# ubc-vision/StableKeypoints

Hardware: AMD Instinct MI355X
Metric: images/sec for token-optimization step (SD1.5, 512^2, K=10 kpts) (higher is better)
Workload: dtype f32 (fp32 MFMA / VALU throughout; flash attention of the >= 1024-key self-attention layers: 3xbf16 operand split, fp32 accumulate, error <= the fp32 kernel's)

## Files before the change

### include/skp.h

```cpp
#ifndef SKP_H
#define SKP_H

#include <stdint.h>

#ifdef __cplusplus
extern "C" {
#endif

#define SKP_MAX_LAYERS 8
#define SKP_MAX_SUBJECTS 4

#define SKP_E_BADARG (-1)
#define SKP_E_RANGE  (-2)
#define SKP_E_LDS    (-3)

int skp_abi_version(void);

int skp_tune_set(const char* key, int value);
int skp_tune_get(const char* key);

int skp_gemm_nt_f32(const float* A, const float* B, float* C, int M, int N, int K, int Z0, int Z1,
                    int64_t sa0, int64_t sa1, int64_t sam, int64_t sak,
                    int64_t sb0, int64_t sb1, int64_t sbn, int64_t sbk,
                    int64_t sc0, int64_t sc1, int64_t scm, float alpha, void* stream);
// ... 32 lines not shown
int skp_unwarp_accumulate_f32(const float* M, const float* theta_inv, int n, int K, int R, int S, float* tot, float* num,
                              int finish, void* stream);

int skp_group_norm_coef_f32(const float* x, const float* off, const float* gamma, const float* beta, float* mean, float* rstd,
                            float* coef, const float* bs, int nblk, int pix, float* workspace, int N, int C, int G, int HW,
                            float eps, void* stream);
int skp_conv3x3_f4_gn_ok(int B, int Cin, int Cout, int H, int W);
int skp_conv3x3_f4_gn_f32(const void* x, const void* U, const void* bias, const void* residual, void* y, float* stats,
                          const float* coef, int B, int Cin, int Cout, int H, int W, void* stream);

int skp_conv3x3_f4r_ok(int B, int Cin, int Cout, int H, int W);
int skp_conv3x3_f4r_filter_f32(const void* w, void* R, int Cout, int Cin, int flip_transpose, void* stream);
int64_t skp_conv3x3_f4r_workspace(int B, int Cin, int Cout, int H, int W);
int skp_conv3x3_f4r_f32(const void* x, const void* R, const void* bias, const void* residual, void* y, void* workspace,
                        int B, int Cin, int Cout, int H, int W, void* stream);

int skp_cross_attn_fwd_f32(const float* q, const float* k, const float* v, float* out, float* lse,
                           int B, int Bk, int H, int N, int T, int d, float scale, void* stream);
int64_t skp_cross_attn_bwd_workspace(int B, int H, int N, int T, int d);
int skp_cross_attn_bwd_f32(const float* q, const float* k, const float* v, const float* out,
                           const float* dout, const float* lse, float* dq, float* dk, float* dv,
                           float* workspace, int B, int Bk, int H, int N, int T, int d, float scale,
                           void* stream);

int skp_text_attn_fwd_ok(int B, int H, int N, int d, int ld);
int skp_text_attn_fwd_f32(const float* q, const float* k, const float* v, float* out,
                          int B, int H, int N, int d, int ld, float scale, void* stream);

int skp_attn_map_bwd_ex_f32(const float* const* S , float* const* dS , const int* s ,
                            int L, int B, int H, int T, int R, const float* dM, const float* lse,
                            float* workspace, float* dot_io, int ldt, int64_t m_bstride, int mode, void* stream);

int64_t skp_flash_attn_bwd_workspace(int B, int Bk, int H, int N, int Nk, int d);
int skp_flash_attn_fwd_f32(const float* q, const float* k, const float* v, float* out, float* lse,
                           int B, int Bk, int H, int N, int Nk, int d, float scale, void* stream);
int skp_flash_attn_bwd_f32(const float* q, const float* k, const float* v, const float* out, const float* dout,
                           const float* lse, float* dq, float* dk, float* dv, float* workspace,
                           int B, int Bk, int H, int N, int Nk, int d, float scale, void* stream);
int skp_flash_attn_bwd_ld_f32(const float* q, const float* k, const float* v, const float* out, const float* dout,
                              const float* lse, float* dq, float* dk, float* dv, float* workspace,
                              int B, int Bk, int H, int N, int Nk, int d, float scale, int ldg, void* stream);

int skp_flash_attn_fwd_split_ok(int B, int Bk, int H, int N, int Nk, int d);
int64_t skp_flash_attn_fwd_split_workspace(int B, int Bk, int H, int N, int Nk, int d);
int skp_flash_attn_fwd_split_f32(const float* q, const float* k, const float* v, float* out, float* lse, void* workspace,
                                 int B, int Bk, int H, int N, int Nk, int d, float scale, void* stream);
// ... 128 lines not shown
```

### stablekeypoints_amd/_native.py

```python
from __future__ import annotations

import ctypes as C
import os

import torch

_HERE = os.path.dirname(os.path.abspath(__file__))
LIB_PATH = os.environ.get("SKP_LIB_PATH") or os.path.join(_HERE, "csrc", "libskp_hip.so")
ABI_VERSION = 44

_vp, _i, _f, _i64 = C.c_void_p, C.c_int, C.c_float, C.c_int64

SIGNATURES = {
    "skp_abi_version": [],
    "skp_tune_set": [C.c_char_p, _i],
    "skp_tune_get": [C.c_char_p],
    "skp_group_norm_onepass_ok": [_i, _i, _i, _i],
    "skp_gemm_nt_f32": [_vp, _vp, _vp, _i, _i, _i, _i, _i,
                        _i64, _i64, _i64, _i64, _i64, _i64, _i64, _i64, _i64, _i64, _i64, _f, _vp],
    "skp_qk_logits_f32": [_vp, _vp, _vp, _i, _i, _i, _i, _i, _i, _f, _vp],
    "skp_attn_map_fwd_f32": [C.POINTER(_vp), C.POINTER(_i), _i, _i, _i, _i, _i, _vp, _vp, _vp],
    "skp_attn_map_fwd_ex_f32": [C.POINTER(_vp), C.POINTER(_i), _i, _i, _i, _i, _i, _vp, _vp, _vp, _i, _i64, _i, _vp],
    "skp_attn_map_bwd_ex_f32": [C.POINTER(_vp), C.POINTER(_vp), C.POINTER(_i), _i, _i, _i, _i, _i, _vp, _vp, _vp, _vp,
                                _i, _i64, _i, _vp],
    "skp_attn_map_bwd_workspace": [C.POINTER(_i), _i, _i, _i, _i, _i],
    "skp_attn_map_bwd_f32": [C.POINTER(_vp), C.POINTER(_vp), C.POINTER(_i), _i, _i, _i, _i, _i, _vp, _vp, _vp, _vp],
    "skp_group_norm_coef_f32": [_vp, _vp, _vp, _vp, _vp, _vp, _vp, _vp, _i, _i, _vp, _i, _i, _i, _i, _f, _vp],
    "skp_conv3x3_f4_gn_ok": [_i, _i, _i, _i, _i],
    "skp_conv3x3_f4_gn_f32": [_vp, _vp, _vp, _vp, _vp, _vp, _vp, _i, _i, _i, _i, _i, _vp],
    "skp_unwarp_accumulate_f32": [_vp, _vp, _i, _i, _i, _i, _vp, _vp, _i, _vp],
    "skp_attn_map_fwd_wide_f32": [C.POINTER(_vp), C.POINTER(_i), _i, _i, _i, _i, _i, _vp, _vp, _vp, _i, _i, _vp],
    "skp_attn_map_fwd_wide_ok": [C.POINTER(_i), _i, _i, _i],
    "skp_attn_map_bwd_col_ok": [C.POINTER(_i), _i, _i, _i, _i, _i],
    "skp_attn_map_bwd_col_workspace": [C.POINTER(_i), _i, _i, _i, _i, _i, _i],
    "skp_attn_map_bwd_col_f32": [C.POINTER(_vp), C.POINTER(_vp), C.POINTER(_i), _i, _i, _i, _i, _i, _vp, _vp, _i, _vp, _vp,
                                 _i, _vp],
    "skp_attn_map_bwd_sparse_workspace": [C.POINTER(_i), _i, _i, _i, _i, _i, _i],
    "skp_attn_map_bwd_sparse_f32": [C.POINTER(_vp), C.POINTER(_vp), C.POINTER(_i), _i, _i, _i, _i, _i, _vp, _vp, _i, _vp, _vp,
                                    _i, _vp],
    "skp_token_stats_f32": [_vp, _i, _i, _i, _f, _f, _vp, _vp, _vp, _vp],
    "skp_select_tokens": [_vp, _vp, _i, _i, _i, _i, _vp, _vp, _vp],
    "skp_select_tokens_batched": [_vp, _vp, _i, _i, _i, _i, _i, _vp, _vp, _vp],
    "skp_losses_fwd_f32": [_vp, _vp, _vp, _i, _i, _i, _vp, _i, _f, C.POINTER(_f), _vp, _vp, _vp, _vp, _vp],
    "skp_losses_fwd_dev_f32": [_vp, _vp, _vp, _i, _i, _i, _vp, _i, _f, _vp, _vp, _vp, _vp, _vp, _vp],
    "skp_rows_axpy_f32": [_vp, _vp, _i, _i64, _vp, _vp, _vp, _vp, _vp],
    "skp_cross_attn_fwd_f32": [_vp, _vp, _vp, _vp, _vp, _i, _i, _i, _i, _i, _i, _f, _vp],
    "skp_cross_attn_bwd_workspace": [_i, _i, _i, _i, _i],
    "skp_cross_attn_bwd_f32": [_vp, _vp, _vp, _vp, _vp, _vp, _vp, _vp, _vp, _vp, _i, _i, _i, _i, _i, _i, _f, _vp],
    "skp_text_attn_fwd_ok": [_i, _i, _i, _i, _i],
    "skp_text_attn_fwd_f32": [_vp, _vp, _vp, _vp, _i, _i, _i, _i, _i, _f, _vp],
    "skp_group_norm_fwd_f32": [_vp, _vp, _vp, _vp, _vp, _vp, _vp, _vp, _i, _i, _i, _i, _f, _i, _vp],
    "skp_group_norm_bwd_f32": [_vp, _vp, _vp, _vp, _vp, _vp, _vp, _vp, _vp, _i, _i, _i, _i, _f, _i, _vp],
    "skp_group_norm_bwd_add_f32": [_vp, _vp, _vp, _vp, _vp, _vp, _vp, _vp, _vp, _vp, _i, _i, _i, _i, _f, _i, _vp],
    "skp_add_bias_residual_f32": [_vp, _vp, _vp, _vp, _i, _i, _i, _vp],
    "skp_add_layer_norm_ok": [_i],
    "skp_add_layer_norm_fwd_f32": [_vp, _vp, _vp, _vp, _vp, _vp, _vp, _i64, _i, _f, _vp],
    "skp_add_layer_norm_bwd_f32": [_vp, _vp, _vp, _vp, _vp, _vp, _i64, _i, _vp],
    "skp_conv3x3_filter_f32": [_vp, _vp, _i, _i, _i, _vp],
    "skp_conv3x3_workspace": [_i, _i, _i, _i, _i, _i],
    "skp_conv3x3_f32": [_vp, _vp, _vp, _vp, _vp, _vp, _i, _i, _i, _i, _i, _i, _vp],
    "skp_conv3x3_f4_filter_f32": [_vp, _vp, _i, _i, _i, _vp],
    "skp_conv3x3_f4_workspace": [_i, _i, _i, _i, _i],
    "skp_conv3x3_f4_f32": [_vp, _vp, _vp, _vp, _vp, _vp, _i, _i, _i, _i, _i, _vp],
    "skp_flash_attn_fwd_split_ok": [_i, _i, _i, _i, _i, _i],
    "skp_flash_attn_fwd_split_workspace": [_i, _i, _i, _i, _i, _i],
    "skp_flash_attn_fwd_split_f32": [_vp, _vp, _vp, _vp, _vp, _vp, _i, _i, _i, _i, _i, _i, C.c_float, _vp],
    "skp_flash_attn_fwd_wide_ok": [_i, _i, _i, _i, _i, _i],
    "skp_flash_attn_fwd_wide_workspace": [_i, _i, _i, _i, _i, _i],
    "skp_flash_attn_fwd_wide_f32": [_vp, _vp, _vp, _vp, _vp, _i, _i, _i, _i, _i, _i, _f, _vp],
    "skp_flash_attn_bwd_split_ok": [_i, _i, _i, _i, _i, _i],
    "skp_flash_attn_bwd_split_workspace": [_i, _i, _i, _i, _i, _i],
# ... 120 lines not shown
```

### stablekeypoints_amd/csrc/skp_common.h

```cpp
#pragma once
#include <hip/hip_runtime.h>
#include <stdint.h>
#include "../../include/skp.h"

#define SKP_WAVE 64
#define SKP_LOG2E 1.4426950408889634f

typedef float f32x16 __attribute__((ext_vector_type(16)));
typedef float f32x4 __attribute__((ext_vector_type(4)));
typedef float f32x2 __attribute__((ext_vector_type(2)));

enum { SKP_TUNE_WINO_SPLIT = 0, SKP_TUNE_WINO_RAW_MAX_TILES, SKP_TUNE_MAP_BANDS, SKP_TUNE_FA2_TWO_KERNEL_BWD, SKP_TUNE_GN_FOLD_MAX_COUT, SKP_TUNE_CROSS_ATTN_TS,
       SKP_TUNE_CONV_S2W, SKP_TUNE_CONV_UP2, SKP_TUNE_COUNT };
int skp_tune(int key);

static inline int skp_launch_status() {
    hipError_t e = hipGetLastError();
    return e == hipSuccess ? 0 : (int)e;
}

__device__ __forceinline__ void skp_cubic_taps(int dst, float ratio, int n, int idx[4], float w[4]) {
    const float A = -0.75f;
    const float src = ratio * ((float)dst + 0.5f) - 0.5f;
    const float fl = floorf(src);
    const float t = src - fl;
    const int i0 = (int)fl;
    float x = t + 1.0f;
    w[0] = ((A * x - 5.0f * A) * x + 8.0f * A) * x - 4.0f * A;
    x = t;
    w[1] = ((A + 2.0f) * x - (A + 3.0f)) * x * x + 1.0f;
    x = 1.0f - t;
    w[2] = ((A + 2.0f) * x - (A + 3.0f)) * x * x + 1.0f;
    x = 2.0f - t;
    w[3] = ((A * x - 5.0f * A) * x + 8.0f * A) * x - 4.0f * A;
#pragma unroll
    for (int i = 0; i < 4; ++i) {
// ... 44 lines not shown
```

### stablekeypoints_amd/csrc/skp_cross_attn.hip

```cpp
#include "skp_attn_tiles.h"

#define SKP_CA_KSPLIT_MAX 16

int skp_gemm_nt_splitk(const float* A, const float* B, float* C, float* partial, int64_t c_elems, int ksplit,
                       int M, int N, int K, int Z0, int Z1,
                       int64_t sa0, int64_t sa1, int64_t sam, int64_t sak,
                       int64_t sb0, int64_t sb1, int64_t sbn, int64_t sbk,
                       int64_t sc0, int64_t sc1, int64_t scm, float alpha, void* stream);

static int ca_ksplit(int N) { int k = N / 256; return k < 1 ? 1 : (k > SKP_CA_KSPLIT_MAX ? SKP_CA_KSPLIT_MAX : k); }

template <int D8, int TT>
__global__ __launch_bounds__(256) void skp_cross_attn_fwd_kernel(const float* __restrict__ q, const float* __restrict__ k,
                                                                 const float* __restrict__ v, float* __restrict__ out,
                                                                 float* __restrict__ lse, int Bk, int H, int N, int T,
                                                                 float scale) {
    using S = CAShape<D8, TT>;
    extern __shared__ __attribute__((aligned(16))) float smem[];
    const int tid = threadIdx.x, wave = tid >> 6, lane = tid & 63, i = lane & 31, hi = lane >> 5;
    const int b = blockIdx.z, h = blockIdx.y, C = H * S::D;
    const int n0 = blockIdx.x * 128 + wave * 32, n = n0 + i;
    const bool nv = n < N;
    const float* qrow = q + ((size_t)b * N + (nv ? n : N - 1)) * C + h * S::D;
    const float sl2 = scale * SKP_LOG2E;
    f32x4 qv[D8];
#pragma unroll
    for (int j = 0; j < D8; ++j) qv[j] = *(const f32x4*)(qrow + 8 * j + 4 * hi) * sl2;
    const size_t kvoff = (Bk == 1 ? 0 : (size_t)b * T * C) + (size_t)h * S::D;
    ca_stage<D8, TT>(smem, k + kvoff, T, C, tid);
    __syncthreads();
    f32x16 acc[TT];
// ... 37 lines not shown
                const int nn = n0 + (r & 3) + 8 * (r >> 2) + 4 * hi;
                if (nn < N) out[((size_t)b * N + nn) * C + h * S::D + c] = o[ct][r];
            }
        }
    }
}

template <int D8, int TT>
__global__ __launch_bounds__(256) void skp_cross_attn_bwd_kernel(const float* __restrict__ q, const float* __restrict__ k,
                                                                 const float* __restrict__ v, const float* __restrict__ out,
                                                                 const float* __restrict__ dout, const float* __restrict__ lse,
                                                                 float* __restrict__ dq, float* __restrict__ Pst,
                                                                 float* __restrict__ dSst, int Bk, int H, int N, int T,
                                                                 float scale) {
    using S = CAShape<D8, TT>;
    extern __shared__ __attribute__((aligned(16))) float smem[];
    const int tid = threadIdx.x, wave = tid >> 6, lane = tid & 63, i = lane & 31, hi = lane >> 5;
    const int b = blockIdx.z, h = blockIdx.y, C = H * S::D;
    const int n0 = blockIdx.x * 128 + wave * 32, n = n0 + i;
    const bool nv = n < N;
    const size_t rowoff = ((size_t)b * N + (nv ? n : N - 1)) * C + h * S::D;
    const float sl2 = scale * SKP_LOG2E;
    const size_t kvoff = (Bk == 1 ? 0 : (size_t)b * T * C) + (size_t)h * S::D;
    ca_stage<D8, TT>(smem, k + kvoff, T, C, tid);
    f32x16 p[TT], dp[TT];
    float dsum = 0.f;
    {
        f32x4 qv[D8];
#pragma unroll
        for (int j = 0; j < D8; ++j) qv[j] = *(const f32x4*)(q + rowoff + 8 * j + 4 * hi) * sl2;
        __syncthreads();
#pragma unroll
        for (int tt = 0; tt < TT; ++tt)
#pragma unroll
            for (int r = 0; r < 16; ++r) p[tt][r] = 0.f;
        ca_swapped_product<D8, TT>(smem, qv, p, i, hi);
    }
    const float lse2 = lse[((size_t)b * H + h) * N + (nv ? n : N - 1)] * SKP_LOG2E;
#pragma unroll
    for (int tt = 0; tt < TT; ++tt)
#pragma unroll
        for (int r = 0; r < 16; ++r)
            p[tt][r] = (ca_tok(tt, r, hi) < T) ? __builtin_amdgcn_exp2f(p[tt][r] - lse2) : 0.f;
    __syncthreads();
    ca_stage<D8, TT>(smem, v + kvoff, T, C, tid);
    {
        f32x4 dov[D8];
#pragma unroll
        for (int j = 0; j < D8; ++j) {
            dov[j] = *(const f32x4*)(dout + rowoff + 8 * j + 4 * hi);
            const f32x4 ov = *(const f32x4*)(out + rowoff + 8 * j + 4 * hi);
            dsum += dov[j][0] * ov[0] + dov[j][1] * ov[1] + dov[j][2] * ov[2] + dov[j][3] * ov[3];
        }
        dsum += __shfl_xor(dsum, 32, 64);
        __syncthreads();
#pragma unroll
        for (int tt = 0; tt < TT; ++tt)
#pragma unroll
            for (int r = 0; r < 16; ++r) dp[tt][r] = 0.f;
        ca_swapped_product<D8, TT>(smem, dov, dp, i, hi);
    }
    const size_t stb = ((size_t)b * H + h) * S::TP * N;
#pragma unroll
    for (int tt = 0; tt < TT; ++tt)
#pragma unroll
        for (int r = 0; r < 16; ++r) {
            dp[tt][r] = p[tt][r] * (dp[tt][r] - dsum);
            if (nv) {
                const size_t o = stb + (size_t)ca_tok(tt, r, hi) * N + n;
                Pst[o] = p[tt][r];
                dSst[o] = dp[tt][r];
            }
        }
    __syncthreads();
    ca_stage<D8, TT>(smem, k + kvoff, T, C, tid);
    __syncthreads();
    f32x16 o[S::CT];
    ca_reg_product<D8, TT>(smem, dp, o, i, hi);
#pragma unroll
    for (int ct = 0; ct < S::CT; ++ct) {
        const int c = ct * 32 + i;
        if (c < S::D) {
#pragma unroll
            for (int r = 0; r < 16; ++r) {
                const int nn = n0 + (r & 3) + 8 * (r >> 2) + 4 * hi;
                if (nn < N) dq[((size_t)b * N + nn) * C + h * S::D + c] = scale * o[ct][r];
            }
        }
    }
}

template <int D8>
struct CATS {
    using S = CAShape<D8, 1>;
    static constexpr int OUT = S::CT * 1024;
    static constexpr int REG = (32 * S::LDK > OUT ? 32 * S::LDK : OUT);
};

template <int D8>
// ... 126 lines not shown
        ca_swapped_product<D8, 1>(reg, qv, p, i, hi);
    }
    const float lse2 = lse[((size_t)b * H + h) * N + (nv ? n : N - 1)] * SKP_LOG2E;
#pragma unroll
    for (int r = 0; r < 16; ++r) p[0][r] = (t0 + ca_tok(0, r, hi) < T) ? __builtin_amdgcn_exp2f(p[0][r] - lse2) : 0.f;
    ca_stage_wave<D8>(reg, v + kvoff, t0, T, C, lane);
    {
        f32x4 dov[D8];
#pragma unroll
        for (int j = 0; j < D8; ++j) {
            dov[j] = *(const f32x4*)(dout + rowoff + 8 * j + 4 * hi);
            const f32x4 ov = *(const f32x4*)(out + rowoff + 8 * j + 4 * hi);
            dsum += dov[j][0] * ov[0] + dov[j][1] * ov[1] + dov[j][2] * ov[2] + dov[j][3] * ov[3];
        }
        dsum += __shfl_xor(dsum, 32, 64);
#pragma unroll
        for (int r = 0; r < 16; ++r) dp[0][r] = 0.f;
        ca_swapped_product<D8, 1>(reg, dov, dp, i, hi);
    }
    const size_t stb = ((size_t)b * H + h) * TP * N;
#pragma unroll
    for (int r = 0; r < 16; ++r) {
        dp[0][r] = p[0][r] * (dp[0][r] - dsum);
        if (nv) {
            const size_t o = stb + (size_t)(t0 + ca_tok(0, r, hi)) * N + n;
            Pst[o] = p[0][r];
            dSst[o] = dp[0][r];
        }
    }
    ca_stage_wave<D8>(reg, k + kvoff, t0, T, C, lane);
    f32x16 o[S::CT];
    ca_reg_product<D8, 1>(reg, dp, o, i, hi);
    ca_merge_store<D8, NW>(smem, reg, o, dq, scale, b, h, H, N, n0, wave, lane);
}

static bool ca_use_ts(int B, int H, int N, int T, int d) {
    if (skp_tune(SKP_TUNE_CROSS_ATTN_TS) == 1) return false;
    const int tt = (T + 31) / 32;
    if (tt < 2 || !(d == 80 || d == 160)) return false;
    return (long)((N + 127) / 128) * H * B * 4 < 1024;
}

static int ca_check(int B, int Bk, int H, int N, int T, int d) {
    if (B <= 0 || H <= 0 || N <= 0 || T <= 0 || d <= 0 || (Bk != 1 && Bk != B)) return SKP_E_BADARG;
    if (T > 128 || B > 65535 || H > 65535) return SKP_E_RANGE;
    if (d != 8 && d != 16 && d != 32 && d != 40 && d != 64 && d != 80 && d != 160) return SKP_E_RANGE;
    return 0;
}

#define SKP_CA_DISPATCH(KERNEL, ...)                                                                     \
    {                                                                                                    \
        const int tt = (T + 31) / 32;                                                                    \
        const int tsel = tt <= 1 ? 1 : (tt <= 3 ? 3 : 4);                                                \
        dim3 grid((N + 127) / 128, H, B), block(256);                                                    \
        hipStream_t st = (hipStream_t)stream;                                                            \
        int launched = 0;                                                                                \
        SKP_CA_CASE(KERNEL, 1, 1, __VA_ARGS__) SKP_CA_CASE(KERNEL, 1, 3, __VA_ARGS__) SKP_CA_CASE(KERNEL, 1, 4, __VA_ARGS__)     \
        SKP_CA_CASE(KERNEL, 2, 1, __VA_ARGS__) SKP_CA_CASE(KERNEL, 2, 3, __VA_ARGS__) SKP_CA_CASE(KERNEL, 2, 4, __VA_ARGS__)     \
        SKP_CA_CASE(KERNEL, 4, 1, __VA_ARGS__) SKP_CA_CASE(KERNEL, 4, 3, __VA_ARGS__) SKP_CA_CASE(KERNEL, 4, 4, __VA_ARGS__)     \
        SKP_CA_CASE(KERNEL, 5, 1, __VA_ARGS__) SKP_CA_CASE(KERNEL, 5, 3, __VA_ARGS__) SKP_CA_CASE(KERNEL, 5, 4, __VA_ARGS__)     \
        SKP_CA_CASE(KERNEL, 8, 1, __VA_ARGS__) SKP_CA_CASE(KERNEL, 8, 3, __VA_ARGS__) SKP_CA_CASE(KERNEL, 8, 4, __VA_ARGS__)     \
        SKP_CA_CASE(KERNEL, 10, 1, __VA_ARGS__) SKP_CA_CASE(KERNEL, 10, 3, __VA_ARGS__) SKP_CA_CASE(KERNEL, 10, 4, __VA_ARGS__)  \
        SKP_CA_CASE(KERNEL, 20, 1, __VA_ARGS__) SKP_CA_CASE(KERNEL, 20, 3, __VA_ARGS__) SKP_CA_CASE(KERNEL, 20, 4, __VA_ARGS__)  \
        if (!launched) return SKP_E_RANGE;                                                               \
    }

#define SKP_CA_CASE(KERNEL, D8V, TTV, ...)                                                               \
    if (!launched && d == D8V * 8 && tsel == TTV) {                                                      \
        const size_t lds = CAShape<D8V, TTV>::LDS_FLOATS * sizeof(float);                                \
        if (lds > 64 * 1024) {                                                                           \
            hipError_t e = hipFuncSetAttribute((const void*)KERNEL<D8V, TTV>,                            \
                                               hipFuncAttributeMaxDynamicSharedMemorySize, (int)lds);    \
            if (e != hipSuccess) return (int)e;                                                          \
        }                                                                                                \
        hipLaunchKernelGGL((KERNEL<D8V, TTV>), grid, block, lds, st, __VA_ARGS__);                       \
        launched = 1;                                                                                    \
    }

#define SKP_CA_TS_CASE(KERNEL, D8V, NWV, ...)                                                            \
    if (!launched && d == D8V * 8 && nw == NWV) {                                                        \
        const size_t lds = ((size_t)NWV * CATS<D8V>::REG + 2 * NWV * 32) * sizeof(float);                \
        if (lds > 64 * 1024) {                                                                           \
            hipError_t e = hipFuncSetAttribute((const void*)KERNEL<D8V, NWV>,                            \
                                               hipFuncAttributeMaxDynamicSharedMemorySize, (int)lds);    \
            if (e != hipSuccess) return (int)e;                                                          \
        }                                                                                                \
        hipLaunchKernelGGL((KERNEL<D8V, NWV>), dim3((N + 31) / 32, H, B), dim3(64 * NWV), lds, (hipStream_t)stream, __VA_ARGS__); \
        launched = 1;                                                                                    \
    }
#define SKP_CA_TS_DISPATCH(KERNEL, ...)                                                                  \
    {                                                                                                    \
        const int nw = (T + 31) / 32 <= 3 ? ((T + 31) / 32 <= 2 ? 2 : 3) : 4;                            \
// ... 6 lines not shown
extern "C" int skp_cross_attn_tp(int T) {
    const int tt = (T + 31) / 32;
    return (tt <= 1 ? 1 : (tt <= 3 ? 3 : 4)) * 32;
}

extern "C" int64_t skp_cross_attn_bwd_workspace(int B, int H, int N, int T, int d) {
    if (B <= 0 || H <= 0 || N <= 0 || T <= 0 || T > 128 || d <= 0) return SKP_E_BADARG;
    return (2 * (int64_t)B * H * skp_cross_attn_tp(T) * N + (int64_t)ca_ksplit(N) * B * T * H * d) * (int64_t)sizeof(float);
}

extern "C" int skp_cross_attn_fwd_f32(const float* q, const float* k, const float* v, float* out, float* lse,
                                      int B, int Bk, int H, int N, int T, int d, float scale, void* stream) {
    if (!q || !k || !v || !out || !lse) return SKP_E_BADARG;
    int rc = ca_check(B, Bk, H, N, T, d);
    if (rc) return rc;
    if (ca_use_ts(B, H, N, T, d)) {
        SKP_CA_TS_DISPATCH(skp_cross_attn_fwd_ts_kernel, q, k, v, out, lse, Bk, H, N, T, scale)
        return skp_launch_status();
    }
    SKP_CA_DISPATCH(skp_cross_attn_fwd_kernel, q, k, v, out, lse, Bk, H, N, T, scale)
    return skp_launch_status();
}

extern "C" int skp_cross_attn_bwd_f32(const float* q, const float* k, const float* v, const float* out,
                                      const float* dout, const float* lse, float* dq, float* dk, float* dv,
                                      float* workspace, int B, int Bk, int H, int N, int T, int d, float scale,
                                      void* stream) {
    if (!q || !k || !v || !out || !dout || !lse || !dq || !dk || !dv || !workspace) return SKP_E_BADARG;
    int rc = ca_check(B, Bk, H, N, T, d);
    if (rc) return rc;
    const int TP = skp_cross_attn_tp(T);
    float* Pst = workspace;
    float* dSst = workspace + (size_t)B * H * TP * N;
    if (ca_use_ts(B, H, N, T, d)) {
        SKP_CA_TS_DISPATCH(skp_cross_attn_bwd_ts_kernel, q, k, v, out, dout, lse, dq, Pst, dSst, Bk, H, N, T, TP, scale)
    } else {
        SKP_CA_DISPATCH(skp_cross_attn_bwd_kernel, q, k, v, out, dout, lse, dq, Pst, dSst, Bk, H, N, T, scale)
    }
    rc = skp_launch_status();
    if (rc) return rc;
    const int64_t C = (int64_t)H * d;
    float* part = dSst + (size_t)B * H * TP * N;
    const int ksp = ca_ksplit(N);
    const int64_t celems = (int64_t)B * T * C;
    rc = skp_gemm_nt_splitk(dSst, q, dk, part, celems, ksp, T, d, N, B, H, (int64_t)H * TP * N, (int64_t)TP * N, N, 1,
                            (int64_t)N * C, d, 1, C, (int64_t)T * C, d, C, scale, stream);
    if (rc) return rc;
    return skp_gemm_nt_splitk(Pst, dout, dv, part, celems, ksp, T, d, N, B, H, (int64_t)H * TP * N, (int64_t)TP * N, N, 1,
                              (int64_t)N * C, d, 1, C, (int64_t)T * C, d, C, 1.0f, stream);
}
```

### stablekeypoints_amd/csrc/skp_select_loss.hip

```cpp
#include "skp_common.h"
#include <string.h>

__device__ __forceinline__ bool skp_better(float v, int i, float bv, int bi) {
    return (v > bv) || (v == bv && i < bi);
}

struct StatsArgs { int T, R, S; float sigma, eps; };

__global__ __launch_bounds__(256) void skp_token_stats_kernel(const float* __restrict__ M, StatsArgs a,
                                                              int32_t* __restrict__ argmax_out,
                                                              float* __restrict__ kl_out, float* __restrict__ ent_out) {
    __shared__ float red_v[4];
    __shared__ int red_i[4];
    __shared__ float red[4];
    __shared__ float s_cy[SKP_MAX_SUBJECTS], s_cx[SKP_MAX_SUBJECTS];
    const int t = blockIdx.x, tid = threadIdx.x, R = a.R, RR = R * R;
    const float* m = M + (size_t)t * RR;
    const float rad = 0.05f * (float)R;
    const float rad2 = rad * rad;
    float maxval0 = 0.f;
    for (int j = 0; j < a.S; ++j) {
        float bv = -INFINITY; int bi = 0x7fffffff;
        for (int p = tid; p < RR; p += 256) {
            const int row = p / R, col = p - row * R;
// ... 348 lines not shown
}

__global__ __launch_bounds__(256) void skp_rows_axpy_kernel(float* __restrict__ dst, const int64_t* __restrict__ sel,
                                                            int64_t n, const float* __restrict__ x,
                                                            const float* __restrict__ a, const float* __restrict__ y,
                                                            const float* __restrict__ b) {
    const int k = blockIdx.y;
    const int64_t i = (int64_t)blockIdx.x * 256 + threadIdx.x;
    if (i >= n) return;
    float v = a[0] * x[(size_t)k * n + i];
    if (y) v += b[0] * y[(size_t)k * n + i];
    dst[(size_t)sel[k] * n + i] += v;
}

extern "C" int skp_rows_axpy_f32(float* dst, const int64_t* sel, int K, int64_t n, const float* x, const float* a,
                                 const float* y, const float* b, void* stream) {
    if (!dst || !sel || !x || !a || K <= 0 || n <= 0 || (y && !b)) return SKP_E_BADARG;
    if (K > 65535) return SKP_E_RANGE;
    hipLaunchKernelGGL(skp_rows_axpy_kernel, dim3((unsigned)((n + 255) / 256), K), dim3(256), 0, (hipStream_t)stream,
                       dst, sel, n, x, a, y, b);
    return skp_launch_status();
}

extern "C" int skp_abi_version(void) { return 44; }

static int g_tune[SKP_TUNE_COUNT] = {0};
static const char* const g_tune_names[SKP_TUNE_COUNT] = {"wino_split", "wino_raw_max_tiles", "map_bands", "fa2_two_kernel_bwd", "gn_fold_max_cout", "cross_attn_ts", "conv_s2w", "conv_up2"};
int skp_tune(int key) { return (key >= 0 && key < SKP_TUNE_COUNT) ? g_tune[key] : 0; }
extern "C" int skp_tune_set(const char* key, int value) {
    if (!key || value < 0) return SKP_E_BADARG;
    for (int i = 0; i < SKP_TUNE_COUNT; ++i)
        if (!strcmp(key, g_tune_names[i])) { g_tune[i] = value; return 0; }
    return SKP_E_RANGE;
}
extern "C" int skp_tune_get(const char* key) {
    if (!key) return SKP_E_BADARG;
    for (int i = 0; i < SKP_TUNE_COUNT; ++i)
        if (!strcmp(key, g_tune_names[i])) return g_tune[i];
    return SKP_E_RANGE;
}
```

### stablekeypoints_amd/ops.py

```python
from __future__ import annotations

import contextlib
import weakref
from typing import List, Sequence, Tuple

import torch

from . import _native as N
from . import routes


def _stream() -> int:
    return torch.cuda.current_stream().cuda_stream


def _dev(t: torch.Tensor, name: str) -> torch.Tensor:
    if not t.is_cuda:
        raise RuntimeError(f"{name}: the StableKeypoints hot path runs on the HIP kernels only "
                           f"(got a {t.device} tensor; there is no CPU fallback)")
    if t.dtype != torch.float32:
        raise RuntimeError(f"{name}: expected float32, got {t.dtype}")
    return t if t.is_contiguous() else t.contiguous()


# ... 502 lines not shown
    @staticmethod
    def forward(ctx, q, k, v, heads: int, scale: float):
        q, k, v = _dev(q, "q"), _dev(k, "k"), _dev(v, "v")
        B, Nq, C = q.shape
        Bk, T, _ = k.shape
        out = torch.empty_like(q)
        lse = torch.empty(B, heads, Nq, device=q.device, dtype=torch.float32)
        routes.note("attn.cross", routes.cross_attn_form(B, heads, Nq, T, C // heads, N.lib().skp_tune_get(b"cross_attn_ts") == 1))
        N.check(N.lib().skp_cross_attn_fwd_f32(q.data_ptr(), k.data_ptr(), v.data_ptr(), out.data_ptr(), lse.data_ptr(),
                                               B, Bk, heads, Nq, T, C // heads, float(scale), _stream()),
                "skp_cross_attn_fwd_f32")
        ctx.save_for_backward(q, k, v, out, lse)
        ctx.meta = (heads, float(scale))
        return out

    @staticmethod
    def backward(ctx, dout):
        q, k, v, out, lse = ctx.saved_tensors
        heads, scale = ctx.meta
        dout = _dev(dout, "dout")
        B, Nq, C = q.shape
        Bk, T, _ = k.shape
        dq = torch.empty_like(q)
        dk = torch.empty(B, T, C, device=q.device, dtype=torch.float32)
        dv = torch.empty_like(dk)
        ws = _workspace("skp_cross_attn_bwd_workspace", B, heads, Nq, T, C // heads, device=q.device)
        N.check(N.lib().skp_cross_attn_bwd_f32(q.data_ptr(), k.data_ptr(), v.data_ptr(), out.data_ptr(), dout.data_ptr(),
                                               lse.data_ptr(), dq.data_ptr(), dk.data_ptr(), dv.data_ptr(), _ptr(ws),
                                               B, Bk, heads, Nq, T, C // heads, scale, _stream()),
                "skp_cross_attn_bwd_f32")
        if Bk == 1 and B > 1:
            dk, dv = dk.sum(dim=0, keepdim=True), dv.sum(dim=0, keepdim=True)
        return dq, dk, dv, None, None


def cross_attention(q, k, v, heads: int, scale: float):
    if k.shape[1] > CROSS_ATTN_MAX_T:
        routes.note("attn.cross", "flash")
        return FlashAttnFn.apply(q, k, v, int(heads), float(scale))
    return CrossAttnFn.apply(q, k, v, int(heads), float(scale))


TEXT_ATTN_MODE = "auto"
TEXT_ATTN_MODES = ("auto", "lib")


def text_attn_supported(width: int, heads: int, n_tokens: int) -> bool:
    return (width % heads == 0
            and N.lib().skp_text_attn_fwd_ok(1, int(heads), int(n_tokens), int(width) // int(heads), int(width)) == 1)


def _text_attn_lib(q, k, v, heads: int, scale: float):
    B, Nn, C = q.shape
    qh, kh, vh = (t.reshape(B, Nn, heads, C // heads).permute(0, 2, 1, 3) for t in (q, k, v))
    S = torch.matmul(qh, kh.transpose(-1, -2)) * scale
# ... 1042 lines not shown
```

Baseline: 54.11.

## Add fused dK/dV reduction kernel for cross-attention backward with batch folding

Adds a dedicated MFMA kernel that computes dK and dV together from the stored P and dS tiles, with partial sums split across N chunks, plus a combine kernel that folds batch partials into a single Bk=1 gradient. This replaces two split-K GEMMs and a host-side torch sum over the batch dimension. For d=40/80 with TT=3, the backward stage also stages K and V into LDS once up front, dropping the restaging and extra barriers. The cost is more LDS per block and a larger workspace for the partials.

After: 54.36 (median of 6 runs). No clear change (+0.5%).

```diff
diff --git a/include/skp.h b/include/skp.h
--- a/include/skp.h
+++ b/include/skp.h
@@ -78,6 +78,11 @@
                            const float* dout, const float* lse, float* dq, float* dk, float* dv,
                            float* workspace, int B, int Bk, int H, int N, int T, int d, float scale,
                            void* stream);
+int64_t skp_cross_attn_bwd_rows_workspace(int B, int H, int N, int T, int d);
+int skp_cross_attn_bwd_rows_f32(const float* q, const float* k, const float* v, const float* out,
+                                const float* dout, const float* lse, float* dq, float* dk, float* dv,
+                                float* workspace, int B, int Bk, int H, int N, int T, int d, float scale,
+                                void* stream);
 
 int skp_text_attn_fwd_ok(int B, int H, int N, int d, int ld);
 int skp_text_attn_fwd_f32(const float* q, const float* k, const float* v, float* out,
diff --git a/stablekeypoints_amd/_native.py b/stablekeypoints_amd/_native.py
--- a/stablekeypoints_amd/_native.py
+++ b/stablekeypoints_amd/_native.py
@@ -7,7 +7,7 @@
 
 _HERE = os.path.dirname(os.path.abspath(__file__))
 LIB_PATH = os.environ.get("SKP_LIB_PATH") or os.path.join(_HERE, "csrc", "libskp_hip.so")
-ABI_VERSION = 44
+ABI_VERSION = 45
 
 _vp, _i, _f, _i64 = C.c_void_p, C.c_int, C.c_float, C.c_int64
 
@@ -47,6 +47,8 @@
     "skp_cross_attn_fwd_f32": [_vp, _vp, _vp, _vp, _vp, _i, _i, _i, _i, _i, _i, _f, _vp],
     "skp_cross_attn_bwd_workspace": [_i, _i, _i, _i, _i],
     "skp_cross_attn_bwd_f32": [_vp, _vp, _vp, _vp, _vp, _vp, _vp, _vp, _vp, _vp, _i, _i, _i, _i, _i, _i, _f, _vp],
+    "skp_cross_attn_bwd_rows_workspace": [_i, _i, _i, _i, _i],
+    "skp_cross_attn_bwd_rows_f32": [_vp, _vp, _vp, _vp, _vp, _vp, _vp, _vp, _vp, _vp, _i, _i, _i, _i, _i, _i, _f, _vp],
     "skp_text_attn_fwd_ok": [_i, _i, _i, _i, _i],
     "skp_text_attn_fwd_f32": [_vp, _vp, _vp, _vp, _i, _i, _i, _i, _i, _f, _vp],
     "skp_group_norm_fwd_f32": [_vp, _vp, _vp, _vp, _vp, _vp, _vp, _vp, _i, _i, _i, _i, _f, _i, _vp],
diff --git a/stablekeypoints_amd/csrc/skp_common.h b/stablekeypoints_amd/csrc/skp_common.h
--- a/stablekeypoints_amd/csrc/skp_common.h
+++ b/stablekeypoints_amd/csrc/skp_common.h
@@ -11,7 +11,7 @@
 typedef float f32x2 __attribute__((ext_vector_type(2)));
 
 enum { SKP_TUNE_WINO_SPLIT = 0, SKP_TUNE_WINO_RAW_MAX_TILES, SKP_TUNE_MAP_BANDS, SKP_TUNE_FA2_TWO_KERNEL_BWD, SKP_TUNE_GN_FOLD_MAX_COUT, SKP_TUNE_CROSS_ATTN_TS,
-       SKP_TUNE_CONV_S2W, SKP_TUNE_CONV_UP2, SKP_TUNE_COUNT };
+       SKP_TUNE_CONV_S2W, SKP_TUNE_CONV_UP2, SKP_TUNE_CROSS_ATTN_DKV, SKP_TUNE_COUNT };
 int skp_tune(int key);
 
 static inline int skp_launch_status() {
diff --git a/stablekeypoints_amd/csrc/skp_cross_attn.hip b/stablekeypoints_amd/csrc/skp_cross_attn.hip
--- a/stablekeypoints_amd/csrc/skp_cross_attn.hip
+++ b/stablekeypoints_amd/csrc/skp_cross_attn.hip
@@ -7,6 +7,15 @@
                        int64_t sa0, int64_t sa1, int64_t sam, int64_t sak,
                        int64_t sb0, int64_t sb1, int64_t sbn, int64_t sbk,
                        int64_t sc0, int64_t sc1, int64_t scm, float alpha, void* stream);
+
+template <int D8, int TT>
+constexpr bool ca_kv_once() { return (D8 == 5 || D8 == 10) && TT == 3; }
+template <int D8, int TT>
+constexpr size_t skp_cross_attn_fwd_kernel_lds() { return CAShape<D8, TT>::LDS_FLOATS * sizeof(float); }
+template <int D8, int TT>
+constexpr size_t skp_cross_attn_bwd_kernel_lds() {
+    return (CAShape<D8, TT>::LDS_FLOATS + (ca_kv_once<D8, TT>() ? CAShape<D8, TT>::TP * CAShape<D8, TT>::LDK : 0)) * sizeof(float);
+}
 
 static int ca_ksplit(int N) { int k = N / 256; return k < 1 ? 1 : (k > SKP_CA_KSPLIT_MAX ? SKP_CA_KSPLIT_MAX : k); }
 
@@ -90,7 +99,10 @@
     const size_t rowoff = ((size_t)b * N + (nv ? n : N - 1)) * C + h * S::D;
     const float sl2 = scale * SKP_LOG2E;
     const size_t kvoff = (Bk == 1 ? 0 : (size_t)b * T * C) + (size_t)h * S::D;
+    constexpr bool KV2 = ca_kv_once<D8, TT>();
+    float* smv = KV2 ? smem + S::TP * S::LDK : smem;
     ca_stage<D8, TT>(smem, k + kvoff, T, C, tid);
+    if (KV2) ca_stage<D8, TT>(smv, v + kvoff, T, C, tid);
     f32x16 p[TT], dp[TT];
     float dsum = 0.f;
     {
@@ -110,8 +122,10 @@
 #pragma unroll
         for (int r = 0; r < 16; ++r)
             p[tt][r] = (ca_tok(tt, r, hi) < T) ? __builtin_amdgcn_exp2f(p[tt][r] - lse2) : 0.f;
-    __syncthreads();
-    ca_stage<D8, TT>(smem, v + kvoff, T, C, tid);
+    if (!KV2) {
+        __syncthreads();
+        ca_stage<D8, TT>(smem, v + kvoff, T, C, tid);
+    }
     {
         f32x4 dov[D8];
 #pragma unroll
@@ -121,12 +135,12 @@
             dsum += dov[j][0] * ov[0] + dov[j][1] * ov[1] + dov[j][2] * ov[2] + dov[j][3] * ov[3];
         }
         dsum += __shfl_xor(dsum, 32, 64);
-        __syncthreads();
+        if (!KV2) __syncthreads();
 #pragma unroll
         for (int tt = 0; tt < TT; ++tt)
 #pragma unroll
             for (int r = 0; r < 16; ++r) dp[tt][r] = 0.f;
-        ca_swapped_product<D8, TT>(smem, dov, dp, i, hi);
+        ca_swapped_product<D8, TT>(smv, dov, dp, i, hi);
     }
     const size_t stb = ((size_t)b * H + h) * S::TP * N;
 #pragma unroll
@@ -134,15 +148,17 @@
 #pragma unroll
         for (int r = 0; r < 16; ++r) {
             dp[tt][r] = p[tt][r] * (dp[tt][r] - dsum);
-            if (nv) {
+            if (nv && ca_tok(tt, r, hi) < T) {
                 const size_t o = stb + (size_t)ca_tok(tt, r, hi) * N + n;
                 Pst[o] = p[tt][r];
                 dSst[o] = dp[tt][r];
             }
         }
-    __syncthreads();
-    ca_stage<D8, TT>(smem, k + kvoff, T, C, tid);
-    __syncthreads();
+    if (!KV2) {
+        __syncthreads();
+        ca_stage<D8, TT>(smem, k + kvoff, T, C, tid);
+        __syncthreads();
+    }
     f32x16 o[S::CT];
     ca_reg_product<D8, TT>(smem, dp, o, i, hi);
 #pragma unroll
@@ -315,7 +331,7 @@
 #pragma unroll
     for (int r = 0; r < 16; ++r) {
         dp[0][r] = p[0][r] * (dp[0][r] - dsum);
-        if (nv) {
+        if (nv && t0 + ca_tok(0, r, hi) < T) {
             const size_t o = stb + (size_t)(t0 + ca_tok(0, r, hi)) * N + n;
             Pst[o] = p[0][r];
             dSst[o] = dp[0][r];
@@ -360,7 +376,7 @@
 
 #define SKP_CA_CASE(KERNEL, D8V, TTV, ...)                                                               \
     if (!launched && d == D8V * 8 && tsel == TTV) {                                                      \
-        const size_t lds = CAShape<D8V, TTV>::LDS_FLOATS * sizeof(float);                                \
+        const size_t lds = KERNEL##_lds<D8V, TTV>();                                                     \
         if (lds > 64 * 1024) {                                                                           \
             hipError_t e = hipFuncSetAttribute((const void*)KERNEL<D8V, TTV>,                            \
                                                hipFuncAttributeMaxDynamicSharedMemorySize, (int)lds);    \
@@ -413,6 +429,29 @@
     return skp_launch_status();
 }
 
+static int ca_bwd_stage(const float* q, const float* k, const float* v, const float* out, const float* dout, const float* lse,
+                        float* dq, float* Pst, float* dSst, int B, int Bk, int H, int N, int T, int TP, int d, float scale,
+                        void* stream) {
+    if (ca_use_ts(B, H, N, T, d)) {
+        SKP_CA_TS_DISPATCH(skp_cross_attn_bwd_ts_kernel, q, k, v, out, dout, lse, dq, Pst, dSst, Bk, H, N, T, TP, scale)
+    } else {
+        SKP_CA_DISPATCH(skp_cross_attn_bwd_kernel, q, k, v, out, dout, lse, dq, Pst, dSst, Bk, H, N, T, scale)
+    }
+    return skp_launch_status();
+}
+
+static int ca_dkv_gemm(const float* q, const float* dout, const float* Pst, const float* dSst, float* part, float* dk, float* dv,
+                       int B, int H, int N, int T, int TP, int d, float scale, void* stream) {
+    const int64_t C = (int64_t)H * d;
+    const int ksp = ca_ksplit(N);
+    const int64_t celems = (int64_t)B * T * C;
+    int rc = skp_gemm_nt_splitk(dSst, q, dk, part, celems, ksp, T, d, N, B, H, (int64_t)H * TP * N, (int64_t)TP * N, N, 1,
+                                (int64_t)N * C, d, 1, C, (int64_t)T * C, d, C, scale, stream);
+    if (rc) return rc;
+    return skp_gemm_nt_splitk(Pst, dout, dv, part, celems, ksp, T, d, N, B, H, (int64_t)H * TP * N, (int64_t)TP * N, N, 1,
+                              (int64_t)N * C, d, 1, C, (int64_t)T * C, d, C, 1.0f, stream);
+}
+
 extern "C" int skp_cross_attn_bwd_f32(const float* q, const float* k, const float* v, const float* out,
                                       const float* dout, const float* lse, float* dq, float* dk, float* dv,
                                       float* workspace, int B, int Bk, int H, int N, int T, int d, float scale,
@@ -423,20 +462,43 @@
     const int TP = skp_cross_attn_tp(T);
     float* Pst = workspace;
     float* dSst = workspace + (size_t)B * H * TP * N;
-    if (ca_use_ts(B, H, N, T, d)) {
-        SKP_CA_TS_DISPATCH(skp_cross_attn_bwd_ts_kernel, q, k, v, out, dout, lse, dq, Pst, dSst, Bk, H, N, T, TP, scale)
-    } else {
-        SKP_CA_DISPATCH(skp_cross_attn_bwd_kernel, q, k, v, out, dout, lse, dq, Pst, dSst, Bk, H, N, T, scale)
-    }
-    rc = skp_launch_status();
-    if (rc) return rc;
-    const int64_t C = (int64_t)H * d;
+    rc = ca_bwd_stage(q, k, v, out, dout, lse, dq, Pst, dSst, B, Bk, H, N, T, TP, d, scale, stream);
+    if (rc) return rc;
+    return ca_dkv_gemm(q, dout, Pst, dSst, dSst + (size_t)B * H * TP * N, dk, dv, B, H, N, T, TP, d, scale, stream);
+}
+
+int64_t skp_cross_attn_dkv_partial_floats(int B, int H, int N, int T, int d);
+int skp_cross_attn_dkv_launch(const float* q, const float* dout, const float* Pst, const float* dSst, float* part, float* dk,
+                              float* dv, int B, int Bk, int H, int N, int T, int TP, int d, float scale, void* stream);
+int skp_cross_attn_dkv_combine(const float* part, float* dk, float* dv, int64_t n, int64_t sstride, int64_t pstride, int nslot,
+                               float scale, void* stream);
+
+extern "C" int64_t skp_cross_attn_bwd_rows_workspace(int B, int H, int N, int T, int d) {
+    if (B <= 0 || H <= 0 || N <= 0 || T <= 0 || T > 128 || d <= 0) return SKP_E_BADARG;
+    const int64_t row = (int64_t)B * T * H * d;
+    const int64_t gemm = ((int64_t)ca_ksplit(N) + 2) * row, tiled = skp_cross_attn_dkv_partial_floats(B, H, N, T, d);
+    return (2 * (int64_t)B * H * skp_cross_attn_tp(T) * N + (gemm > tiled ? gemm : tiled)) * (int64_t)sizeof(float);
+}
+
+extern "C" int skp_cross_attn_bwd_rows_f32(const float* q, const float* k, const float* v, const float* out,
+                                           const float* dout, const float* lse, float* dq, float* dk, float* dv,
+                                           float* workspace, int B, int Bk, int H, int N, int T, int d, float scale,
+                                           void* stream) {
+    if (!q || !k || !v || !out || !dout || !lse || !dq || !dk || !dv || !workspace) return SKP_E_BADARG;
+    int rc = ca_check(B, Bk, H, N, T, d);
+    if (rc) return rc;
+    const int TP = skp_cross_attn_tp(T);
+    float* Pst = workspace;
+    float* dSst = workspace + (size_t)B * H * TP * N;
     float* part = dSst + (size_t)B * H * TP * N;
-    const int ksp = ca_ksplit(N);
-    const int64_t celems = (int64_t)B * T * C;
-    rc = skp_gemm_nt_splitk(dSst, q, dk, part, celems, ksp, T, d, N, B, H, (int64_t)H * TP * N, (int64_t)TP * N, N, 1,
-                            (int64_t)N * C, d, 1, C, (int64_t)T * C, d, C, scale, stream);
-    if (rc) return rc;
-    return skp_gemm_nt_splitk(Pst, dout, dv, part, celems, ksp, T, d, N, B, H, (int64_t)H * TP * N, (int64_t)TP * N, N, 1,
-                              (int64_t)N * C, d, 1, C, (int64_t)T * C, d, C, 1.0f, stream);
-}
+    rc = ca_bwd_stage(q, k, v, out, dout, lse, dq, Pst, dSst, B, Bk, H, N, T, TP, d, scale, stream);
+    if (rc) return rc;
+    if (skp_tune(SKP_TUNE_CROSS_ATTN_DKV) != 2)
+        return skp_cross_attn_dkv_launch(q, dout, Pst, dSst, part, dk, dv, B, Bk, H, N, T, TP, d, scale, stream);
+    if (Bk != 1 || B == 1) return ca_dkv_gemm(q, dout, Pst, dSst, part, dk, dv, B, H, N, T, TP, d, scale, stream);
+    const int64_t n = (int64_t)T * H * d;
+    float* rows = part + (size_t)ca_ksplit(N) * B * n;
+    rc = ca_dkv_gemm(q, dout, Pst, dSst, part, rows, rows + (size_t)B * n, B, H, N, T, TP, d, scale, stream);
+    if (rc) return rc;
+    return skp_cross_attn_dkv_combine(rows, dk, dv, n, n, (int64_t)B * n, B, 1.0f, stream);
+}
diff --git a/stablekeypoints_amd/csrc/skp_cross_attn_dkv.hip b/stablekeypoints_amd/csrc/skp_cross_attn_dkv.hip
--- /dev/null
+++ b/stablekeypoints_amd/csrc/skp_cross_attn_dkv.hip
@@ -0,0 +1,236 @@
+#include "skp_common.h"
+
+namespace {
+
+template <int D, int TT, bool CSPLIT>
+struct DKV {
+    static constexpr int LDK = D + 4, CT = (D + 15) / 16, Q4 = D / 4;
+    static constexpr int NB = 2, NR = 16 * NB;
+    static constexpr int U = NR * Q4 / 64;
+    static constexpr int REG = NR * LDK + 16;
+    static constexpr int STEP = CSPLIT ? NR : 2 * NR;
+    static constexpr int MERGE = CSPLIT ? 0 : TT * CT * 256;
+    static constexpr int LDS_FLOATS = 4 * REG > MERGE ? 4 * REG : MERGE;
+};
+
+}
+
+template <int D, int TT, bool CSPLIT>
+__global__ __launch_bounds__(256) void skp_cross_attn_dkv_kernel(const float* __restrict__ q, const float* __restrict__ dout,
+                                                                 const float* __restrict__ Pst, const float* __restrict__ dSst,
+                                                                 float* __restrict__ part, int Bk, int H, int N, int T, int TP,
+                                                                 int dfull, int P, int L) {
+    using K = DKV<D, TT, CSPLIT>;
+    extern __shared__ __attribute__((aligned(16))) float smem[];
+    const int tid = threadIdx.x, wave = tid >> 6, lane = tid & 63, i16 = lane & 15, g = lane >> 4;
+    const int pr = wave & 1, hf = wave >> 1;
+    const int b = blockIdx.x / P, chunk = blockIdx.x - b * P, h = blockIdx.y;
+    const int C = H * dfull;
+    const int n_lo = chunk * L, n_hi = min(N, n_lo + L);
+    const int choff = h * dfull + (CSPLIT ? hf * D : 0);
+    const float* X = (pr ? dout : q) + (size_t)b * N * C + choff;
+    const float* St = (pr ? Pst : dSst) + ((size_t)b * H + h) * TP * N;
+    float* reg = smem + wave * K::REG;
+    const bool al = (N & 3) == 0;
+
+    int goff[K::U], loff[K::U], xrow[K::U];
+#pragma unroll
+    for (int u = 0; u < K::U; ++u) {
+        const int idx = lane + 64 * u;
+        const int row = idx / K::Q4, c4 = idx - row * K::Q4;
+        xrow[u] = row;
+        goff[u] = row * C + 4 * c4;
+        loff[u] = row * K::LDK + 4 * c4;
+    }
+    auto load_st = [&](f32x4 (&s)[K::NB][TT], int nw) {
+#pragma unroll
+        for (int nb = 0; nb < K::NB; ++nb)
+#pragma unroll
+            for (int tt = 0; tt < TT; ++tt) {
+                const int t = 16 * tt + i16, n = nw + 16 * nb + 4 * g;
+                f32x4 v = {0.f, 0.f, 0.f, 0.f};
+                if (t < T && n < n_hi) {
+                    const float* p = St + (size_t)t * N + n;
+                    if (al) {
+                        v = *(const f32x4*)p;
+                    } else {
+#pragma unroll
+                        for (int e = 0; e < 4; ++e)
+                            if (n + e < n_hi) v[e] = p[e];
+                    }
+                }
+                s[nb][tt] = v;
+            }
+    };
+    auto fetch_x = [&](f32x4 (&x)[K::U], int nw) {
+        const float* src = X + (size_t)nw * C;
+#pragma unroll
+        for (int u = 0; u < K::U; ++u) {
+            x[u] = f32x4{0.f, 0.f, 0.f, 0.f};
+            if (nw + xrow[u] < n_hi) x[u] = *(const f32x4*)(src + goff[u]);
+        }
+    };
+
+    f32x4 acc[K::CT][TT];
+#pragma unroll
+    for (int ct = 0; ct < K::CT; ++ct)
+#pragma unroll
+        for (int tt = 0; tt < TT; ++tt) acc[ct][tt] = f32x4{0.f, 0.f, 0.f, 0.f};
+
+    const int nw0 = n_lo + (CSPLIT ? 0 : hf * K::NR);
+    f32x4 sc[K::NB][TT], sn[K::NB][TT], xr[K::U];
+    load_st(sc, nw0);
+    fetch_x(xr, nw0);
+    for (int nw = nw0; nw < n_hi; nw += K::STEP) {
+#pragma unroll
+        for (int u = 0; u < K::U; ++u) *(f32x4*)(reg + loff[u]) = xr[u];
+        __builtin_amdgcn_fence(__ATOMIC_RELEASE, "wavefront");
+        __builtin_amdgcn_wave_barrier();
+        __builtin_amdgcn_fence(__ATOMIC_ACQUIRE, "wavefront");
+        const bool more = nw + K::STEP < n_hi;
+        if (more) {
+            load_st(sn, nw + K::STEP);
+            fetch_x(xr, nw + K::STEP);
+        }
+#pragma unroll
+        for (int nb = 0; nb < K::NB; ++nb)
+#pragma unroll
+            for (int r = 0; r < 4; ++r) {
+                const float* row = reg + (16 * nb + 4 * g + r) * K::LDK + i16;
+#pragma unroll
+                for (int ct = 0; ct < K::CT; ++ct) {
+                    const float a = row[16 * ct];
+#pragma unroll
+                    for (int tt = 0; tt < TT; ++tt)
+                        acc[ct][tt] = __builtin_amdgcn_mfma_f32_16x16x4f32(a, sc[nb][tt][r], acc[ct][tt], 0, 0, 0);
+                }
+            }
+        __builtin_amdgcn_fence(__ATOMIC_RELEASE, "wavefront");
+        __builtin_amdgcn_wave_barrier();
+        __builtin_amdgcn_fence(__ATOMIC_ACQUIRE, "wavefront");
+        if (more) {
+#pragma unroll
+            for (int nb = 0; nb < K::NB; ++nb)
+#pragma unroll
+                for (int tt = 0; tt < TT; ++tt) sc[nb][tt] = sn[nb][tt];
+        }
+    }
+
+    if (!CSPLIT) {
+        __syncthreads();
+#pragma unroll
+        for (int ph = 0; ph < 2; ++ph) {
+            if (pr == ph && hf == 1) {
+#pragma unroll
+                for (int ct = 0; ct < K::CT; ++ct)
+#pragma unroll
+                    for (int tt = 0; tt < TT; ++tt) *(f32x4*)(smem + ((ct * TT + tt) * 64 + lane) * 4) = acc[ct][tt];
+            }
+            __syncthreads();
+            if (pr == ph && hf == 0) {
+#pragma unroll
+                for (int ct = 0; ct < K::CT; ++ct)
+#pragma unroll
+                    for (int tt = 0; tt < TT; ++tt) acc[ct][tt] += *(const f32x4*)(smem + ((ct * TT + tt) * 64 + lane) * 4);
+            }
+            __syncthreads();
+        }
+        if (hf) return;
+    }
+    const int slot = Bk == 1 ? blockIdx.x : chunk, bo = Bk == 1 ? 0 : b;
+    float* pbase = part + (((size_t)slot * 2 + pr) * Bk + bo) * T * C + choff;
+#pragma unroll
+    for (int tt = 0; tt < TT; ++tt) {
+        const int t = 16 * tt + i16;
+        if (t < T) {
+#pragma unroll
+            for (int ct = 0; ct < K::CT; ++ct) {
+                const int c0 = 16 * ct + 4 * g;
+                if (c0 < D) *(f32x4*)(pbase + (size_t)t * C + c0) = acc[ct][tt];
+            }
+        }
+    }
+}
+
+__global__ __launch_bounds__(64) void skp_cross_attn_dkv_combine_kernel(const float* __restrict__ part, float* __restrict__ dk,
+                                                                         float* __restrict__ dv, long n4, long sstride,
+                                                                         long pstride, int nslot, float scale) {
+    const int z = blockIdx.y;
+    const long i = (long)blockIdx.x * 64 + threadIdx.x;
+    if (i >= n4) return;
+    const float* p = part + (size_t)z * pstride + 4 * i;
+    f32x4 acc = *(const f32x4*)p;
+    int s = 1;
+    for (; s + 8 <= nslot; s += 8) {
+        f32x4 v[8];
+#pragma unroll
+        for (int u = 0; u < 8; ++u) v[u] = *(const f32x4*)(p + (size_t)(s + u) * sstride);
+#pragma unroll
+        for (int u = 0; u < 8; ++u) acc += v[u];
+    }
+    for (; s < nslot; ++s) acc += *(const f32x4*)(p + (size_t)s * sstride);
+    ((f32x4*)(z ? dv : dk))[i] = z ? acc : acc * scale;
+}
+
+void skp_cross_attn_dkv_plan(int B, int H, int N, int d, int* P, int* L) {
+    const int step = d == 160 ? 32 : 64;
+    const long rows = (long)B * H;
+    const int perb = rows >= 512 ? 1 : (int)(512 / rows);
+    int l = ((N + perb - 1) / perb + step - 1) / step * step;
+    const int nr = (N + step - 1) / step * step;
+    const int lfloor = d == 160 ? 128 : 256;
+    const int lmin = nr < lfloor ? nr : lfloor;
+    if (l < lmin) l = lmin;
+    *L = l;
+    *P = (N + l - 1) / l;
+}
+
+int64_t skp_cross_attn_dkv_partial_floats(int B, int H, int N, int T, int d) {
+    int P, L;
+    skp_cross_attn_dkv_plan(B, H, N, d, &P, &L);
+    return (int64_t)B * P * 2 * T * H * d;
+}
+
+int skp_cross_attn_dkv_combine(const float* part, float* dk, float* dv, int64_t n, int64_t sstride, int64_t pstride, int nslot,
+                               float scale, void* stream) {
+    const long n4 = (long)(n / 4);
+    hipLaunchKernelGGL(skp_cross_attn_dkv_combine_kernel, dim3((unsigned)((n4 + 63) / 64), 2), dim3(64), 0, (hipStream_t)stream,
+                       part, dk, dv, n4, (long)sstride, (long)pstride, nslot, scale);
+    return skp_launch_status();
+}
+
+#define SKP_DKV_CASE(DV, TTV, CS)                                                                                      \
+    if (!launched && dk_ == DV && tsel == TTV && csplit == CS) {                                                       \
+        const size_t lds = DKV<DV, TTV, CS>::LDS_FLOATS * sizeof(float);                                               \
+        if (lds > 64 * 1024) {                                                                                         \
+            hipError_t e = hipFuncSetAttribute((const void*)skp_cross_attn_dkv_kernel<DV, TTV, CS>,                    \
+                                               hipFuncAttributeMaxDynamicSharedMemorySize, (int)lds);                  \
+            if (e != hipSuccess) return (int)e;                                                                        \
+        }                                                                                                              \
+        hipLaunchKernelGGL((skp_cross_attn_dkv_kernel<DV, TTV, CS>), grid, dim3(256), lds, (hipStream_t)stream, q, dout, Pst,  \
+                           dSst, part, Bk, H, N, T, TP, d, P, L);                                                      \
+        launched = 1;                                                                                                  \
+    }
+#define SKP_DKV_ROW(DV, CS)                                                                                            \
+    SKP_DKV_CASE(DV, 1, CS) SKP_DKV_CASE(DV, 2, CS) SKP_DKV_CASE(DV, 4, CS) SKP_DKV_CASE(DV, 5, CS) SKP_DKV_CASE(DV, 6, CS)   \
+    SKP_DKV_CASE(DV, 8, CS)
+
+int skp_cross_attn_dkv_launch(const float* q, const float* dout, const float* Pst, const float* dSst, float* part, float* dk,
+                              float* dv, int B, int Bk, int H, int N, int T, int TP, int d, float scale, void* stream) {
+    int P, L;
+    skp_cross_attn_dkv_plan(B, H, N, d, &P, &L);
+    if ((long)B * P > 0x7fffffffL / 2 || (long)TP * N > 0x7fffffffL / 4) return SKP_E_RANGE;
+    const int t16 = (T + 15) / 16;
+    const int tsel = t16 <= 2 ? t16 : (t16 <= 4 ? 4 : (t16 <= 6 ? t16 : 8));
+    const bool csplit = d == 160;
+    const int dk_ = csplit ? 80 : d;
+    dim3 grid(B * P, H);
+    int launched = 0;
+    SKP_DKV_ROW(8, false) SKP_DKV_ROW(16, false) SKP_DKV_ROW(32, false) SKP_DKV_ROW(40, false) SKP_DKV_ROW(64, false)
+    SKP_DKV_ROW(80, false) SKP_DKV_ROW(80, true)
+    if (!launched) return SKP_E_RANGE;
+    int rc = skp_launch_status();
+    if (rc) return rc;
+    const int64_t C = (int64_t)H * d, n = (int64_t)Bk * T * C;
+    return skp_cross_attn_dkv_combine(part, dk, dv, n, 2 * n, n, Bk == 1 ? B * P : P, scale, stream);
+}
diff --git a/stablekeypoints_amd/csrc/skp_select_loss.hip b/stablekeypoints_amd/csrc/skp_select_loss.hip
--- a/stablekeypoints_amd/csrc/skp_select_loss.hip
+++ b/stablekeypoints_amd/csrc/skp_select_loss.hip
@@ -394,10 +394,10 @@
     return skp_launch_status();
 }
 
-extern "C" int skp_abi_version(void) { return 44; }
+extern "C" int skp_abi_version(void) { return 45; }
 
 static int g_tune[SKP_TUNE_COUNT] = {0};
-static const char* const g_tune_names[SKP_TUNE_COUNT] = {"wino_split", "wino_raw_max_tiles", "map_bands", "fa2_two_kernel_bwd", "gn_fold_max_cout", "cross_attn_ts", "conv_s2w", "conv_up2"};
+static const char* const g_tune_names[SKP_TUNE_COUNT] = {"wino_split", "wino_raw_max_tiles", "map_bands", "fa2_two_kernel_bwd", "gn_fold_max_cout", "cross_attn_ts", "conv_s2w", "conv_up2", "cross_attn_dkv"};
 int skp_tune(int key) { return (key >= 0 && key < SKP_TUNE_COUNT) ? g_tune[key] : 0; }
 extern "C" int skp_tune_set(const char* key, int value) {
     if (!key || value < 0) return SKP_E_BADARG;
diff --git a/stablekeypoints_amd/ops.py b/stablekeypoints_amd/ops.py
--- a/stablekeypoints_amd/ops.py
+++ b/stablekeypoints_amd/ops.py
@@ -548,15 +548,13 @@
         B, Nq, C = q.shape
         Bk, T, _ = k.shape
         dq = torch.empty_like(q)
-        dk = torch.empty(B, T, C, device=q.device, dtype=torch.float32)
+        dk = torch.empty(Bk, T, C, device=q.device, dtype=torch.float32)
         dv = torch.empty_like(dk)
-        ws = _workspace("skp_cross_attn_bwd_workspace", B, heads, Nq, T, C // heads, device=q.device)
-        N.check(N.lib().skp_cross_attn_bwd_f32(q.data_ptr(), k.data_ptr(), v.data_ptr(), out.data_ptr(), dout.data_ptr(),
-                                               lse.data_ptr(), dq.data_ptr(), dk.data_ptr(), dv.data_ptr(), _ptr(ws),
-                                               B, Bk, heads, Nq, T, C // heads, scale, _stream()),
-                "skp_cross_attn_bwd_f32")
-        if Bk == 1 and B > 1:
-            dk, dv = dk.sum(dim=0, keepdim=True), dv.sum(dim=0, keepdim=True)
+        ws = _workspace("skp_cross_attn_bwd_rows_workspace", B, heads, Nq, T, C // heads, device=q.device)
+        N.check(N.lib().skp_cross_attn_bwd_rows_f32(q.data_ptr(), k.data_ptr(), v.data_ptr(), out.data_ptr(), dout.data_ptr(),
+                                                    lse.data_ptr(), dq.data_ptr(), dk.data_ptr(), dv.data_ptr(), _ptr(ws),
+                                                    B, Bk, heads, Nq, T, C // heads, scale, _stream()),
+                "skp_cross_attn_bwd_rows_f32")
         return dq, dk, dv, None, None
 
 
```
